# markdl/mtcp

Hardware: AMD Instinct MI355X
Metric: device-resident Gpkt/s + payload GB/s checksummed, 1/2/4/8 MI355X (higher is better)
Workload: dtype u8

## Files before the change

### mtcp_amd/csrc/rx_kernels.hpp

```cpp
#pragma once

#include <hip/hip_runtime.h>
#include <stdint.h>

#include <type_traits>

#include "../../include/mtcp_gpu.h"

namespace mg {

constexpr int kWave = 64;
constexpr int kBlock = 256;
constexpr int kWavesPerBlock = kBlock / kWave;
constexpr int kRssTableWords = 24 * 16;
constexpr int kSlotChunks = 8;
constexpr int kRow = 16;
constexpr int kUnroll = 6;

enum Mode : int { kRxChunk = 0, kRxPtrs = 1, kTxChunk = 2, kTxPtrs = 3 };
constexpr bool is_tx(int m) { return m == kTxChunk || m == kTxPtrs; }
enum Sched : int {
    kSchedRolled = 0,
    kSchedUnrolled = 3,
    kSchedSortedBase = 4,
    kSchedSortedEarly = 5,
    kSchedSorted = 6,
};

struct KParams {
    const uint8_t *buf;
    uint64_t buf_len;
    int64_t base_sub;
    const mtcp_gpu_desc *desc;
    const uint8_t *const *ptrs;
    const uint16_t *lens;
    uint32_t n;
    uint32_t off_shift;
    mtcp_gpu_result *out;
    const uint32_t *rss_tables;
    uint32_t rss_nq;
    uint32_t rss_endian;
    uint32_t *fill_count;
    uint32_t *bins;
    uint2 *tx_report;
    uint32_t *stamps;
    uint32_t rss_key[4];
    uint32_t compact;
};

typedef unsigned int v4u __attribute__((ext_vector_type(4)));

typedef __attribute__((address_space(1))) const v4u gv4u;
__device__ __forceinline__ v4u gload(uint64_t addr) { return *reinterpret_cast<gv4u *>(addr); }
__device__ __forceinline__ v4u gload_nt(uint64_t addr) {
    return __builtin_nontemporal_load(reinterpret_cast<gv4u *>(addr));
}
__device__ __forceinline__ uint4 gload4(uint64_t addr) {
    const v4u v = gload(addr);
    return make_uint4(v.x, v.y, v.z, v.w);
}

__device__ __forceinline__ uint32_t bswap16(uint32_t v) {
    return ((v & 0xFFu) << 8) | ((v >> 8) & 0xFFu);
}
__device__ __forceinline__ uint32_t bswap32(uint32_t v) { return __builtin_bswap32(v); }

__device__ __forceinline__ uint32_t halves(uint32_t d, uint32_t acc) {
    return __builtin_amdgcn_sad_u16(d, 0u, acc);
}
__device__ __forceinline__ uint32_t halves4(const v4u &v, uint32_t acc) {
    return halves(v.w, halves(v.z, halves(v.y, halves(v.x, acc))));
}

__device__ __forceinline__ uint32_t fold_csum(uint32_t s) {
    s = (s >> 16) + (s & 0xFFFFu);
    s += s >> 16;
    return (~s) & 0xFFFFu;
}

__device__ __forceinline__ uint32_t row_sum(uint32_t v) {
    v += (uint32_t)__builtin_amdgcn_update_dpp(0, (int)v, 0x111, 0xF, 0xF, true);
    v += (uint32_t)__builtin_amdgcn_update_dpp(0, (int)v, 0x112, 0xF, 0xF, true);
    v += (uint32_t)__builtin_amdgcn_update_dpp(0, (int)v, 0x114, 0xF, 0xF, true);
    v += (uint32_t)__builtin_amdgcn_update_dpp(0, (int)v, 0x118, 0xF, 0xF, true);
    return v;
}

__device__ __forceinline__ uint32_t shfl32(uint32_t v, int src) {
    return (uint32_t)__builtin_amdgcn_ds_bpermute(src << 2, (int)v);
}

__device__ __forceinline__ uint32_t row_bcast(uint32_t v, int i) {
#define MG_NB(n) case n: return (uint32_t)__builtin_amdgcn_update_dpp(0, (int)v, 0x150 + n, 0xF, 0xF, false)
    switch (i) {
        MG_NB(0); MG_NB(1); MG_NB(2); MG_NB(3); MG_NB(4); MG_NB(5); MG_NB(6); MG_NB(7);
        MG_NB(8); MG_NB(9); MG_NB(10); MG_NB(11); MG_NB(12); MG_NB(13); MG_NB(14);
        default: return (uint32_t)__builtin_amdgcn_update_dpp(0, (int)v, 0x15F, 0xF, 0xF, false);
    }
#undef MG_NB
}

__host__ __device__ __forceinline__ uint32_t hash_flow32(const uint32_t (&w)[3]) {
    uint32_t h = 0;
#pragma unroll
    for (int i = 0; i < 12; ++i) {
        h += (uint32_t)(int32_t)(int8_t)(uint8_t)(w[i >> 2] >> (8 * (i & 3)));
        h += h << 10;
        h ^= h >> 6;
    }
    h += h << 3;
    h ^= h >> 11;
    h += h << 15;
    return h;
}

__device__ __forceinline__ uint32_t hash_flow(const uint32_t (&w)[3]) {
    return hash_flow32(w) & (MTCP_GPU_NUM_BINS_FLOWS - 1);
}

__device__ __forceinline__ void flow_key(uint32_t saddr, uint32_t daddr, uint32_t ports, uint32_t (&w)[3]) {
    w[0] = daddr;
    w[1] = saddr;
    w[2] = (ports >> 16) | (ports << 16);
}

__device__ __forceinline__ uint32_t flow_bin(uint32_t saddr, uint32_t daddr, uint32_t ports,
                                             uint32_t verdict) {
    uint32_t w[3];
    flow_key(saddr, daddr, ports, w);
    return verdict == MTCP_GPU_V_TCP_OK ? hash_flow(w) : MTCP_GPU_FLOW_NONE;
}

template <int I0, int N, class F>
__device__ __forceinline__ void static_for(F &&f) {
    if constexpr (I0 < N) {
        f(std::integral_constant<int, I0>{});
        static_for<I0 + 1, N>(f);
    }
}

constexpr int kHdRows = 4 * kSlotChunks;
constexpr int kHdStride = kWave + 1;
struct WaveLds {
    uint32_t hd[kHdRows * kHdStride];
    uint32_t sum[kWave + 1];
    uint4 info[kWave];
};

struct Pkt {
    uint32_t verdict = MTCP_GPU_V_BAD_DESC;
    uint32_t eth_type = 0, ip_len = 0, ihl_doff = 0, ip_csum = 0, tcp_csum = 0;
    uint32_t saddr = 0, daddr = 0, ports = 0, seq = 0, ack = 0, window = 0, flags = 0;
    uint32_t payload_len = 0;
    uint32_t T = 0, s_ip = 0, ip_check = 0;
    uint32_t seg_len = 0;
    uint32_t tcheck = 0;
    bool tcp_entry = false;
    bool need_sum = false;
    bool icmp = false;
};

template <int MODE, class PD, class IPSUM, class SW, class SWB>
__device__ __forceinline__ Pkt parse_head(PD pd, IPSUM ipsum, SW sw, SWB swb, uint32_t L,
                                          bool desc_ok) {
    Pkt k;
    uint32_t h[7];
#pragma unroll
    for (int i = 3; i < 7; ++i) h[i] = pd(i);
    const uint32_t d0 = h[3];
    if (!desc_ok) return k;
    k.verdict = MTCP_GPU_V_TRUNCATED;
    if (L < 14) return k;
    k.eth_type = bswap16(d0 & 0xFFFFu);
    if (k.eth_type != 0x0800u) {
        k.verdict = k.eth_type == 0x0806u ? MTCP_GPU_V_ARP : MTCP_GPU_V_ETH_OTHER;
        return k;
    }
    if (L < 18) return k;
    k.ip_len = bswap16(h[4] & 0xFFFFu);
    const uint32_t ihl = (d0 >> 16) & 0xFu;
    k.ihl_doff = ihl;
    const uint32_t ver = (d0 >> 20) & 0xFu;
    if (!is_tx(MODE) && k.ip_len < 20) {
        k.verdict = MTCP_GPU_V_IP_SHORT;
        return k;
    }
    if (L < 14 + 4 * (ihl > 4 ? ihl : 1)) return k;
    if (ihl >= 5) k.s_ip = ipsum(ihl);
    k.ip_check = h[6] & 0xFFFFu;
    k.ip_csum = ihl <= 4 ? (d0 >> 16) : fold_csum(k.s_ip);
    const uint32_t proto = h[5] >> 24;
    k.T = 14 + 4 * ihl;
    bool tcp_entry = false;
    if (is_tx(MODE)) {
        tcp_entry = ver == 4 && ihl >= 5 && proto == 6 && L >= k.T + 20;
        k.verdict = MTCP_GPU_V_ETH_OTHER;
    } else if (k.ip_csum != 0) {
        k.verdict = MTCP_GPU_V_IP_CSUM_BAD;
    } else if (ver != 4) {
        k.verdict = MTCP_GPU_V_IP_VERSION;
    } else if (proto == 1) {
        k.verdict = MTCP_GPU_V_ICMP;
        if (14 + k.ip_len <= L) {
            if (k.ip_len >= 4 * ihl) {
                k.icmp = k.need_sum = true;
                k.seg_len = k.payload_len = k.ip_len - 4 * ihl;
            } else {
                k.tcp_csum = 0xFFFFu;
            }
        }
    } else if (proto != 6) {
        k.verdict = MTCP_GPU_V_IP_PROTO_OTHER;
    } else if (L >= k.T + 16) {
        tcp_entry = true;
    }
    if (tcp_entry) {
        const uint32_t tw = (k.T - 2) >> 2;
        const uint32_t e3 = pd(tw + 3), e4 = pd(tw + 4);
        const uint32_t doff = (e3 >> 20) & 0xFu;
        k.tcp_entry = true;
        k.saddr = sw(6);
        k.daddr = sw(7);
        k.ports = sw(tw);
        k.seq = swb(tw + 1);
        k.ack = swb(tw + 2);
        k.window = bswap16(e4 & 0xFFFFu);
        k.flags = e3 >> 24;
        k.tcheck = e4 >> 16;
        k.ihl_doff = ihl | (doff << 4);
        if (is_tx(MODE)) {
            if (doff >= 5 && k.ip_len >= 4 * (ihl + doff) && 14 + k.ip_len <= L) {
                k.need_sum = true;
                k.seg_len = k.ip_len - 4 * ihl;
            }
        } else if (k.ip_len < ((ihl + doff) << 2)) {
            k.verdict = MTCP_GPU_V_TCP_LEN_BAD;
        } else {
            k.payload_len = k.ip_len - ((ihl + doff) << 2);
            if (14 + k.ip_len <= L) {
                k.need_sum = true;
                k.seg_len = k.ip_len - 4 * ihl;
            }
        }
    }
    return k;
}

template <int MODE, class PD, class IPSUM, class SW, class SWB>
__device__ __forceinline__ bool parse_common(PD pd, IPSUM ipsum, SW sw, SWB swb, uint32_t L,
                                             bool desc_ok, Pkt &k) {
    if constexpr (is_tx(MODE)) {
        return false;
    } else {
        const uint32_t d0 = pd(3), h4 = pd(4), h5 = pd(5);
        const uint32_t ipl = bswap16(h4 & 0xFFFFu);
        if (!(desc_ok && L >= 50 && (d0 & 0xFFFFFFu) == 0x450008u && (h5 >> 24) == 6u && ipl >= 20u))
            return false;
        const uint32_t s_ip = ipsum(5u);
        if (fold_csum(s_ip) != 0) return false;
        const uint32_t e3 = pd(11), e4 = pd(12);
        const uint32_t doff = (e3 >> 20) & 0xFu, hlen = (5 + doff) << 2;
        const bool len_bad = ipl < hlen;
        k.verdict = len_bad ? MTCP_GPU_V_TCP_LEN_BAD : MTCP_GPU_V_TRUNCATED;
        k.eth_type = 0x0800u;
        k.ip_len = ipl;
        k.ihl_doff = 5u | (doff << 4);
        k.ip_csum = 0;
        k.s_ip = s_ip;
        k.ip_check = pd(6) & 0xFFFFu;
        k.T = 34;
        k.tcp_entry = true;
        k.saddr = sw(6);
        k.daddr = sw(7);
        k.ports = sw(8);
        k.seq = swb(9);
        k.ack = swb(10);
        k.window = bswap16(e4 & 0xFFFFu);
        k.flags = e3 >> 24;
        k.tcheck = e4 >> 16;
        k.payload_len = len_bad ? 0u : ipl - hlen;
        k.need_sum = !len_bad && 14 + ipl <= L;
        k.seg_len = k.need_sum ? ipl - 20 : 0u;
        k.icmp = false;
        k.tcp_csum = 0;
        return true;
    }
}

template <int MODE, class PD, class IPSUM, class SW, class SWB>
__device__ __forceinline__ Pkt parse_head_wave(PD pd, IPSUM ipsum, SW sw, SWB swb, uint32_t L,
                                               bool desc_ok) {
    Pkt k;
    if (parse_common<MODE>(pd, ipsum, sw, swb, L, desc_ok, k)) return k;
    return parse_head<MODE>(pd, ipsum, sw, swb, L, desc_ok);
}

template <int MODE, class PD, class IPSUM, class SW, class SWB>
__device__ __forceinline__ Pkt parse_head_sel(PD pd, IPSUM ipsum, SW sw, SWB swb, uint32_t L,
                                          bool desc_ok) {
    constexpr bool tx = is_tx(MODE);
    const uint32_t d0 = pd(3), h4 = pd(4), h5 = pd(5), h6 = pd(6);
    const uint32_t eth = bswap16(d0 & 0xFFFFu);
    const uint32_t ipl = bswap16(h4 & 0xFFFFu);
    const uint32_t ihl = (d0 >> 16) & 0xFu, ver = (d0 >> 20) & 0xFu;
    const uint32_t proto = h5 >> 24;
    const uint32_t T = 14 + 4 * ihl;
    const bool ok14 = desc_ok && L >= 14;
    const bool isip = ok14 && eth == 0x0800u;
    const bool ok18 = isip && L >= 18;
    const bool shrt = !tx && ipl < 20;
    const bool okhdr = ok18 && !shrt && L >= 14 + 4 * (ihl > 4 ? ihl : 1);
    const uint32_t s_ip = ipsum(ihl);
    const uint32_t ip_csum = ihl <= 4 ? (d0 >> 16) : fold_csum(s_ip);
    const bool ip_good = okhdr && ip_csum == 0 && ver == 4;
    const uint32_t tw = (T - 2) >> 2;
    const uint32_t e3 = pd(tw + 3), e4 = pd(tw + 4);
    const uint32_t doff = (e3 >> 20) & 0xFu;
    const bool tcp_entry = tx ? okhdr && ver == 4 && ihl >= 5 && proto == 6 && L >= T + 20
                              : ip_good && proto == 6 && L >= T + 16;
    const uint32_t hlen = (ihl + doff) << 2;
    const bool in_frame = 14 + ipl <= L;
    const bool len_bad = !tx && tcp_entry && ipl < hlen;
    const bool icmp_in = !tx && ip_good && proto == 1 && in_frame;
    const bool icmp = icmp_in && ipl >= 4 * ihl;
    const bool tcp_sum = tx ? tcp_entry && doff >= 5 && ipl >= hlen && in_frame
                            : tcp_entry && !len_bad && in_frame;

    uint32_t v = MTCP_GPU_V_TRUNCATED;
    if (!tx) {
        v = len_bad ? MTCP_GPU_V_TCP_LEN_BAD : v;
        v = ip_good && proto != 6 ? MTCP_GPU_V_IP_PROTO_OTHER : v;
        v = ip_good && proto == 1 ? MTCP_GPU_V_ICMP : v;
        v = okhdr && ip_csum == 0 && ver != 4 ? MTCP_GPU_V_IP_VERSION : v;
        v = okhdr && ip_csum != 0 ? MTCP_GPU_V_IP_CSUM_BAD : v;
        v = ok18 && shrt ? MTCP_GPU_V_IP_SHORT : v;
    } else {
        v = okhdr ? MTCP_GPU_V_ETH_OTHER : v;
    }
    v = ok14 && !isip ? (eth == 0x0806u ? MTCP_GPU_V_ARP : MTCP_GPU_V_ETH_OTHER) : v;
    v = desc_ok ? v : MTCP_GPU_V_BAD_DESC;

    Pkt k;
    k.verdict = v;
    k.eth_type = ok14 ? eth : 0u;
    k.ip_len = ok18 ? ipl : 0u;
    k.ihl_doff = ok18 ? ihl | (tcp_entry ? doff << 4 : 0u) : 0u;
    k.s_ip = okhdr && ihl >= 5 ? s_ip : 0u;
    k.ip_check = okhdr ? h6 & 0xFFFFu : 0u;
    k.ip_csum = okhdr ? ip_csum : 0u;
    k.T = okhdr ? T : 0u;
    k.tcp_entry = tcp_entry;
    k.saddr = tcp_entry ? sw(6) : 0u;
    k.daddr = tcp_entry ? sw(7) : 0u;
    k.ports = tcp_entry ? sw(tw) : 0u;
    k.seq = tcp_entry ? swb(tw + 1) : 0u;
    k.ack = tcp_entry ? swb(tw + 2) : 0u;
    k.window = tcp_entry ? bswap16(e4 & 0xFFFFu) : 0u;
    k.flags = tcp_entry ? e3 >> 24 : 0u;
    k.tcheck = tcp_entry ? e4 >> 16 : 0u;
    k.icmp = icmp;
    k.need_sum = tcp_sum || icmp;
    k.seg_len = k.need_sum ? ipl - 4 * ihl : 0u;
    k.payload_len = icmp ? ipl - 4 * ihl
                  : !tx && tcp_entry && !len_bad ? ipl - hlen : 0u;
    k.tcp_csum = icmp_in && !icmp ? 0xFFFFu : 0u;
    return k;
}

template <int MODE>
__device__ __forceinline__ void finish_seg(Pkt &k, uint32_t seg) {
    uint32_t s = seg;
    if (is_tx(MODE)) s -= k.tcheck;
    if (!k.icmp) {
        s += (k.saddr & 0xFFFFu) + (k.saddr >> 16);
        s += (k.daddr & 0xFFFFu) + (k.daddr >> 16);
        s += bswap16(k.seg_len);
        s += 0x0600u;
    }
    k.tcp_csum = fold_csum(s);
    if (!is_tx(MODE) && !k.icmp)
        k.verdict = k.tcp_csum ? MTCP_GPU_V_TCP_CSUM_BAD : MTCP_GPU_V_TCP_OK;
}

template <int MODE, int S, bool COMMON = false, bool ALIGNED = false>
__device__ __forceinline__ Pkt parse_finish(const uint32_t *raw, uint32_t sum, uint64_t p,
                                            uint32_t L, uint32_t nch, bool desc_ok) {
    const uint32_t sh = (uint32_t)(p & 15);
    const uint32_t a = sh >> 2, fb = 8 * (sh & 3);
    auto pd = [&](uint32_t i) -> uint32_t {
        if constexpr (ALIGNED) return raw[(a + i) * S];
        return __builtin_amdgcn_alignbit(raw[(a + i + 1) * S], raw[(a + i) * S], fb);
    };
    auto ipsum = [&](uint32_t ihl) -> uint32_t {
        uint32_t s_ip = pd(3) >> 16, lo_last = 0;
#pragma unroll
        for (int j = 1; j < 16; ++j) {
            const uint32_t w = pd(3 + j);
            s_ip = halves(j < (int)ihl ? w : 0u, s_ip);
            lo_last = j == (int)ihl ? w & 0xFFFFu : lo_last;
        }
        return s_ip + lo_last;
    };
    auto sw = [&](uint32_t i) -> uint32_t { return __builtin_amdgcn_alignbit(pd(i + 1), pd(i), 16); };
    auto swb = [&](uint32_t i) -> uint32_t { return bswap32(sw(i)); };
    Pkt k;
    if (!COMMON || !parse_common<MODE>(pd, ipsum, sw, swb, L, desc_ok, k))
        k = parse_head_sel<MODE>(pd, ipsum, sw, swb, L, desc_ok);
    if (k.need_sum) {
        uint32_t s_out = k.s_ip + (pd(3) & 0xFFFFu);
        s_out = halves(pd(2), halves(pd(1), halves(pd(0), s_out)));
#pragma unroll
        for (uint32_t i = 0; i < 3; ++i)
            if (i < a) s_out = halves(raw[i * S], s_out);
        if (!ALIGNED && (sh & 2)) s_out += raw[a * S] & 0xFFFFu;
        const uint64_t p16 = p & ~15ull;
        const uint64_t e_abs = p + 14 + k.ip_len;
        const uint64_t end = p16 + 16ull * nch;
        const uint32_t te = (uint32_t)(e_abs & 15);
        uint64_t cstart = e_abs & ~15ull;
        if (te) {
            uint4 w;
            if (cstart + 16 == end) {
                const uint32_t *t = raw + 4 * (kSlotChunks - 1) * S;
                w = make_uint4(t[0], t[S], t[2 * S], t[3 * S]);
            } else {
                w = gload4(cstart);
            }
            const uint32_t wv[4] = {w.x, w.y, w.z, w.w};
#pragma unroll
            for (int i = 0; i < 4; ++i) {
                const int drop = (int)te - 4 * i;
                const uint32_t m = drop <= 0 ? 0xFFFFFFFFu : drop >= 4 ? 0u : (0xFFFFFFFFu << (8 * drop));
                s_out = halves(wv[i] & m, s_out);
            }
            cstart += 16;
        }
        for (; cstart < end; cstart += 16) {
            const uint4 w = gload4(cstart);
            s_out = halves(w.w, halves(w.z, halves(w.y, halves(w.x, s_out))));
        }
        finish_seg<MODE>(k, sum - s_out);
    }
    return k;
}

__device__ __forceinline__ void pack_record(const Pkt &k, uint32_t rss_hash, uint32_t rss_queue,
                                            uint32_t (&r)[10]) {
    r[0] = k.saddr;
    r[1] = k.daddr;
    r[2] = k.ports;
    r[3] = k.seq;
    r[4] = k.ack;
    r[5] = k.window | (k.ip_len << 16);
    r[6] = k.ip_csum | (k.tcp_csum << 16);
    r[7] = rss_hash;
    r[8] = k.payload_len | (k.ihl_doff << 16) | (k.flags << 24);
    r[9] = k.verdict | (rss_queue << 8) | (k.eth_type << 16);
}

__device__ __forceinline__ void pack_compact(const Pkt &k, uint32_t rss_hash, uint32_t rss_queue,
                                             uint32_t (&r)[4]) {
    r[0] = rss_hash;
    r[1] = k.ip_csum | (k.tcp_csum << 16);
    r[2] = k.payload_len | (k.ip_len << 16);
    r[3] = k.ihl_doff | (k.flags << 8) | (k.verdict << 16) | (rss_queue << 24);
}

__device__ __forceinline__ void store_record(const KParams &kp, uint32_t rec, const Pkt &k,
                                             uint32_t rss_hash, uint32_t rss_queue) {
    if (kp.compact) {
        uint32_t c[4];
        pack_compact(k, rss_hash, rss_queue, c);
        reinterpret_cast<uint4 *>(kp.out)[rec] = make_uint4(c[0], c[1], c[2], c[3]);
    } else {
        uint32_t r[10];
        pack_record(k, rss_hash, rss_queue, r);
        uint2 *o = reinterpret_cast<uint2 *>(kp.out + rec);
#pragma unroll
        for (int i = 0; i < 5; ++i) o[i] = make_uint2(r[2 * i], r[2 * i + 1]);
    }
}

__device__ __forceinline__ uint32_t toeplitz_tables(const uint32_t *tab, uint32_t saddr,
                                                    uint32_t daddr, uint32_t ports) {
    uint32_t hh = 0;
#pragma unroll
    for (int b = 0; b < 4; ++b) {
        const uint32_t sb = (saddr >> (8 * b)) & 0xFFu;
        const uint32_t db = (daddr >> (8 * b)) & 0xFFu;
        const uint32_t pb = (ports >> (8 * b)) & 0xFFu;
        hh ^= tab[((2 * b) << 4) | (sb >> 4)] ^ tab[((2 * b + 1) << 4) | (sb & 15)];
        hh ^= tab[((8 + 2 * b) << 4) | (db >> 4)] ^ tab[((9 + 2 * b) << 4) | (db & 15)];
        hh ^= tab[((16 + 2 * b) << 4) | (pb >> 4)] ^ tab[((17 + 2 * b) << 4) | (pb & 15)];
    }
    return hh;
}

__device__ __forceinline__ uint32_t rss_core(uint32_t hh, uint32_t nq, uint32_t endian) {
    uint32_t m = hh & 0x7Fu;
    if (endian) m ^= 3u;
    return m % nq;
}

struct Frame {
    uint64_t p;
    uint32_t L;
    bool ok, live;
    uint64_t p16;
    uint32_t nch;
    uint32_t r_nch, r_lo, r_hi;
};

struct Trip {
    int i;
    uint32_t c0, nj;
    uint64_t base;
    uint32_t col;
    uint32_t skip = 0;
    uint32_t k = 0, ntrip = 0;
};

template <int MODE, bool RSS, int SCHED, bool LALIGN = false, int ABL = 0, int DEFER = 8, int B = 8,
          bool NT = true, int U = 6, bool REV = false, bool STAMP = false, int PRIO = 0,
          int WPB = kWavesPerBlock, int XSKIP = 0, bool CMP = false, int WPE = 2, bool COOP = true>
__global__ __launch_bounds__(kWave * WPB) __attribute__((amdgpu_waves_per_eu(WPE))) void rx_kernel(KParams kp) {
#ifndef MTCP_GPU_TESTING
    static_assert(ABL == 0 && !STAMP && XSKIP == 0,
                  "rx_kernel's ABL / STAMP / XSKIP variants need a -DMTCP_GPU_TESTING build (tools/)");
#endif
    uint64_t t_start = 0;
    if constexpr (STAMP) t_start = __builtin_amdgcn_s_memrealtime();
    if constexpr ((PRIO & 3) > 0) {
        if (blockIdx.x >= gridDim.x / 2) __builtin_amdgcn_s_setprio(PRIO & 3);
    }
    __shared__ uint32_t rss_lds[RSS ? kRssTableWords : 1];
    __shared__ WaveLds lds[WPB];
    if constexpr (RSS) {
        for (int i = threadIdx.x; i < kRssTableWords; i += kWave * WPB) rss_lds[i] = kp.rss_tables[i];
        __syncthreads();
    }

    const uint32_t lane = threadIdx.x & (kWave - 1);
    const uint32_t row = lane >> 4, rlane = lane & (kRow - 1);
    const uint32_t wib = threadIdx.x >> 6;
    const uint32_t wave = blockIdx.x * WPB + wib;
    const uint32_t nwaves = gridDim.x * WPB;
    WaveLds &wl = lds[wib];
    const uint32_t pass_pkts = nwaves * kWave;
    auto map = [&](uint32_t l) -> uint32_t {
        return B == kWave ? wave * kWave + l : (l / B) * (nwaves * B) + wave * B + (l % B);
    };
    const uint32_t lane_off = map(lane);
    bool xskip_wave = false;
    if constexpr (XSKIP != 0) {
        const uint32_t xcc = (uint32_t)__builtin_amdgcn_s_getreg((3 << 11) | 20) & 1u;
        xskip_wave = XSKIP > 0 ? xcc == 1u : xcc == 0u;
    }
    const uint64_t safe = (uint64_t)(uintptr_t)(MODE == kRxPtrs ? (const void *)kp.out
                                                               : (const void *)kp.buf);
    auto lane_pkt = [&](uint32_t g0, bool &live) -> uint32_t {
        live = g0 + lane_off < kp.n;
        return g0 + lane_off;
    };

    constexpr bool kCoop = B == 8 && MODE != kRxPtrs && SCHED == 3 && COOP;
    __shared__ uint64_t coop_a[kCoop ? 2 : 1][kCoop ? WPB * kWave : 1];
    uint32_t coop_buf = 0;

    const uint32_t cq = wib * kWave + lane, cj = cq / (8 * WPB), cidx = cq % (8 * WPB);
    const uint32_t coop_off = cj * (nwaves * 8) + blockIdx.x * (8 * WPB) + cidx;
    const uint32_t coop_slot = (cidx / 8) * kWave + cj * 8 + (cidx % 8);
    uint64_t raw_a = 0;
    uint32_t raw_b = 0;
    uint64_t cv_a = 0;
    auto fetch = [&](uint32_t g0) {
        if constexpr (kCoop) {
            const uint32_t kk = g0 + coop_off;
            if (kk < kp.n) cv_a = *reinterpret_cast<const uint64_t *>(kp.desc + kk);
            return;
        }
        bool live;
        const uint32_t k = lane_pkt(g0, live);
        if (live) {
            if constexpr (MODE == kRxPtrs) {
                raw_a = (uint64_t)(uintptr_t)kp.ptrs[k];
                raw_b = kp.lens[k];
            } else {
                raw_a = *reinterpret_cast<const uint64_t *>(kp.desc + k);
            }
        }
    };
    auto exchange = [&]() {
        if constexpr (kCoop) {
            coop_a[coop_buf][coop_slot] = cv_a;
            __syncthreads();
            raw_a = coop_a[coop_buf][wib * kWave + lane];
            coop_buf ^= 1u;
        }
    };
    auto decode = [&](uint32_t g0) -> Frame {
        Frame f;
        bool live;
        (void)lane_pkt(g0, live);
        f.live = live;
        if constexpr (XSKIP != 0) {
            if (xskip_wave && g0 + pass_pkts >= kp.n && lane >= (uint32_t)(kWave - (XSKIP > 0 ? XSKIP : -XSKIP)))
                f.live = false;
        }
        f.p = safe;
        f.L = 0;
        f.ok = false;
        if (f.live) {
            if constexpr (MODE == kRxPtrs) {
                f.L = raw_b;
                f.ok = raw_a != 0 && (raw_a & 1) == 0;
                if (f.ok) f.p = raw_a;
            } else {
                const uint32_t off = (uint32_t)raw_a;
                f.L = (uint32_t)(raw_a >> 32) & 0xFFFFu;
                const int64_t pos = (int64_t)((uint64_t)off << kp.off_shift) - kp.base_sub;
                f.ok = pos >= 0 && (pos & 1) == 0 && (uint64_t)pos + f.L <= kp.buf_len;
                if (f.ok) f.p = safe + (uint64_t)pos;
            }
        }
        f.p16 = f.p & ~15ull;
        f.nch = f.ok && f.L ? (uint32_t)((((f.p + f.L + 15) & ~15ull) - f.p16) >> 4) : 0u;
        const int src = 4 * (int)rlane + (int)row;
        f.r_nch = shfl32(f.nch, src);
        f.r_lo = shfl32((uint32_t)f.p16, src);
        f.r_hi = shfl32((uint32_t)(f.p16 >> 32), src);
        return f;
    };

    auto line_align = [&](Trip &t) {
        t.skip = 0;
        if constexpr (LALIGN) {
            if (t.nj > (uint32_t)(U * kRow)) {
                t.skip = (uint32_t)((t.base & 127) >> 4);
                t.base -= 16ull * t.skip;
                t.nj += t.skip;
            }
        }
    };
    auto enter_round = [&](const Frame &f, Trip &t, int ii) {
        t.i = ii;
        t.col = 4 * (uint32_t)ii + row;
        t.nj = row_bcast(f.r_nch, ii);
        t.base = ((uint64_t)row_bcast(f.r_hi, ii) << 32) | row_bcast(f.r_lo, ii);
        t.c0 = 0;
        line_align(t);
        if constexpr (REV) {
            t.k = 0;
            t.ntrip = (t.nj + U * kRow - 1) / (U * kRow);
            if ((row & 1) && t.ntrip > 1) t.c0 = (t.ntrip - 1) * (U * kRow);
        }
    };
    auto rev_step = [&](Trip &t) {
        ++t.k;
        t.c0 = t.k >= t.ntrip ? t.nj
               : (row & 1) ? (t.ntrip - 1 - t.k) * (U * kRow) : t.k * (U * kRow);
    };
    auto advance = [&](const Frame &f, Trip &t) -> bool {
        if (__ballot(t.c0 + U * kRow < t.nj)) {
            t.c0 += U * kRow;
            return true;
        }
        for (int ii = t.i + 1; ii < kWave / 4; ++ii) {
            enter_round(f, t, ii);
            if (__ballot(t.nj != 0)) return true;
        }
        t.nj = 0;
        return false;
    };
    auto first_trip = [&](const Frame &f, Trip &t) -> bool {
        enter_round(f, t, 0);
        return __ballot(t.nj != 0) || advance(f, t);
    };
    auto issue = [&](const Trip &t, v4u (&x)[U]) {
#pragma unroll
        for (int u = 0; u < U; ++u) {
            const uint32_t c = t.c0 + u * kRow + rlane;
            const uint32_t cc = c < t.nj ? c : (t.nj ? t.nj - 1 : 0u);
            x[u] = NT ? gload_nt(t.base + 16ull * cc) : gload(t.base + 16ull * cc);
        }
    };
    auto consume = [&](const Trip &t, const v4u (&x)[U], uint32_t &acc) {
        const uint32_t j = t.col;
        const uint32_t c_hd = rlane - t.skip;
        if (ABL < 2 && t.c0 == 0 && c_hd < kSlotChunks - 1) {
            uint32_t *d = wl.hd + 4 * c_hd * kHdStride + j;
            d[0] = x[0].x; d[kHdStride] = x[0].y;
            d[2 * kHdStride] = x[0].z; d[3 * kHdStride] = x[0].w;
        }
#pragma unroll
        for (int u = 0; u < U; ++u) {
            const uint32_t c = t.c0 + u * kRow + rlane;
            const uint32_t s = halves4(x[u], 0u);
            acc += (ABL >= 3 || c - t.skip < t.nj - t.skip) ? s : 0u;
            if (ABL < 2 && c == t.nj - 1) {
                uint32_t *d = wl.hd + 4 * (kSlotChunks - 1) * kHdStride + j;
                d[0] = x[u].x; d[kHdStride] = x[u].y;
                d[2 * kHdStride] = x[u].z; d[3 * kHdStride] = x[u].w;
            }
        }
    };

    constexpr uint32_t kSmallChunks = 4;
    constexpr uint32_t kQuads = kWave / 4;
    uint32_t pre_nL = 0, pre_nS = 0;
    auto prepare = [&](const Frame &fr, uint32_t &nL, uint32_t &nS) {
        const bool big = fr.nch > kSmallChunks, sml = fr.nch != 0 && !big;
        const uint64_t mb = __ballot(big), ms = __ballot(sml);
        nL = (uint32_t)__popcll(mb);
        nS = (uint32_t)__popcll(ms);
        const uint64_t below = (1ull << lane) - 1;
        const uint4 e = make_uint4((uint32_t)fr.p16, (uint32_t)(fr.p16 >> 32), fr.nch, lane);
        if (big) wl.info[__popcll(mb & below)] = e;
        if (sml) wl.info[kWave - 1 - __popcll(ms & below)] = e;
    };
    auto big_trip = [&](uint32_t nL, uint32_t ii, Trip &t) {
        const uint32_t r = 4 * ii + row;
        t.i = (int)ii;
        t.c0 = 0;
        t.skip = 0;
        t.nj = 0;
        t.base = safe;
        t.col = kWave;
        if (r < nL) {
            const uint4 e = wl.info[r];
            t.base = ((uint64_t)e.y << 32) | e.x;
            t.nj = e.z;
            t.col = e.w;
            line_align(t);
        }
    };
    auto small_trip = [&](uint32_t nS, uint32_t ii, Trip &t) {
        const uint32_t r = kQuads * ii + (lane >> 2);
        t.i = (int)ii;
        t.c0 = 0;
        t.skip = 0;
        t.nj = 0;
        t.base = safe;
        t.col = kWave;
        if (r < nS) {
            const uint4 e = wl.info[kWave - 1 - r];
            t.base = ((uint64_t)e.y << 32) | e.x;
            t.nj = e.z;
            t.col = e.w;
        }
    };
    auto small_load = [&](const Trip &t) -> v4u {
        const uint32_t q = lane & 3;
        const uint32_t cc = q < t.nj ? q : (t.nj ? t.nj - 1 : 0u);
        return NT && SCHED < 5 ? gload_nt(t.base + 16ull * cc) : gload(t.base + 16ull * cc);
    };
    auto small_finish = [&](const Trip &t, const v4u &v) {
        const uint32_t q = lane & 3;
        uint32_t s4 = q < t.nj ? halves4(v, 0u) : 0u;
        s4 += (uint32_t)__builtin_amdgcn_update_dpp(0, (int)s4, 0xB1, 0xF, 0xF, false);
        s4 += (uint32_t)__builtin_amdgcn_update_dpp(0, (int)s4, 0x4E, 0xF, 0xF, false);
        if (q == 0) wl.sum[t.col] = s4;
        if (q < t.nj) {
            uint32_t *d = wl.hd + 4 * q * kHdStride + t.col;
            d[0] = v.x; d[kHdStride] = v.y; d[2 * kHdStride] = v.z; d[3 * kHdStride] = v.w;
        }
        if (q + 1 == t.nj) {
            uint32_t *d = wl.hd + 4 * (kSlotChunks - 1) * kHdStride + t.col;
            d[0] = v.x; d[kHdStride] = v.y; d[2 * kHdStride] = v.z; d[3 * kHdStride] = v.w;
        }
    };

    constexpr int kDefer = MODE == kTxChunk ? 0 : DEFER;
    constexpr int RW = CMP ? 4 : 10, HW = CMP ? 5 : 10;
    uint32_t keep[kDefer > 0 ? kDefer : 1][HW];
    uint32_t held = 0;
    uint32_t last_g0 = 0;
    uint8_t *const out_b = reinterpret_cast<uint8_t *>(kp.out);
    auto flush = [&]() {
        if constexpr (kDefer > 0) {
            static_assert(B % 2 == 0, "16 B pieces need runs of an even number of records");
            constexpr uint32_t kRunDw = B * RW, kRunPieces = kRunDw / 4;
            uint32_t *stg = reinterpret_cast<uint32_t *>(&wl.hd[0]);
#pragma unroll
            for (int q = 0; q < kDefer; ++q) {
                if ((uint32_t)q < held) {
                    const uint32_t gq = last_g0 - (uint32_t)q * pass_pkts;
                    uint2 *st = reinterpret_cast<uint2 *>(stg) + lane * (RW / 2);
#pragma unroll
                    for (int i = 0; i < RW / 2; ++i) st[i] = make_uint2(keep[q][2 * i], keep[q][2 * i + 1]);
#pragma unroll
                    for (uint32_t pc = lane; pc < kWave * RW / 4; pc += kWave) {
                        const uint32_t run = pc / kRunPieces, w = pc % kRunPieces;
                        const uint32_t first = gq + map(run * B);
                        const uint32_t r0 = first + (4 * w) / RW, r1 = first + (4 * w + 2) / RW;
                        const uint4 v = *reinterpret_cast<const uint4 *>(stg + run * kRunDw + 4 * w);
                        uint8_t *dst = out_b + (uint64_t)first * (4 * RW) + 16 * w;
                        if (r1 < kp.n) {
                            *reinterpret_cast<uint4 *>(dst) = v;
                        } else if (r0 < kp.n) {
                            *reinterpret_cast<uint2 *>(dst) = make_uint2(v.x, v.y);
                        }
                    }
                    if (kp.bins) {
                        bool live;
                        const uint32_t rec = lane_pkt(gq, live);
                        if (live)
                            kp.bins[rec] = CMP ? keep[q][HW - 1]
                                               : flow_bin(keep[q][0], keep[q][1], keep[q][2], keep[q][9] & 0xFFu);
                    }
                }
            }
            held = 0;
        }
    };

    auto push = [&](const uint32_t (&r)[HW], uint32_t g0) {
        if constexpr (kDefer > 0) {
            if (held == (uint32_t)kDefer) flush();
#pragma unroll
            for (int q = kDefer - 1; q > 0; --q)
#pragma unroll
                for (int i = 0; i < HW; ++i) keep[q][i] = keep[q - 1][i];
#pragma unroll
            for (int i = 0; i < HW; ++i) keep[0][i] = r[i];
            last_g0 = g0;
            ++held;
        }
    };

    constexpr int kTxDefer = MODE == kTxChunk && DEFER > 0 ? DEFER : 0;
    uint32_t tkeep[kTxDefer > 0 ? kTxDefer : 1][4];
    uint32_t tx_held = 0;
    auto tx_write = [&](const uint32_t (&w)[4]) {
        if (w[3]) {
            uint16_t *q16 = reinterpret_cast<uint16_t *>(((uint64_t)w[1] << 32) | w[0]);
            q16[12] = (uint16_t)w[2];
            q16[(w[3] + 16) >> 1] = (uint16_t)(w[2] >> 16);
        }
    };
    auto tx_flush = [&]() {
        if constexpr (kTxDefer > 0) {
#pragma unroll
            for (int q = 0; q < kTxDefer; ++q)
                if ((uint32_t)q < tx_held) tx_write(tkeep[q]);
            tx_held = 0;
        }
    };
    auto tx_push = [&](const uint32_t (&w)[4]) {
        if constexpr (kTxDefer > 0) {
            if (tx_held == (uint32_t)kTxDefer) tx_flush();
#pragma unroll
            for (int q = kTxDefer - 1; q > 0; --q)
#pragma unroll
                for (int i = 0; i < 4; ++i) tkeep[q][i] = tkeep[q - 1][i];
#pragma unroll
            for (int i = 0; i < 4; ++i) tkeep[0][i] = w[i];
            ++tx_held;
        }
    };

    fetch(0);
    exchange();
    v4u X[U], Y[U];
    Trip pre;
    bool have_pre = false;
    Trip sa, sb;
    v4u va, vb;
    bool have_pre_small = false;
    for (uint32_t g0 = 0; g0 < kp.n; g0 += pass_pkts) {
        if constexpr ((PRIO & 4) != 0) {
            if (g0 == 4 * pass_pkts) __builtin_amdgcn_s_setprio(0);
        }
        const Frame f = decode(g0);
        if (!__ballot(f.live)) break;
        fetch(g0 + pass_pkts);
        const uint32_t k = g0 + lane_off;
        const bool live = f.live, desc_ok = f.ok;
        const uint64_t p = f.p;
        const uint32_t L = f.L, nch = f.nch;
        const bool has_next = g0 + pass_pkts < kp.n;

        if constexpr (SCHED >= 4) {
            uint32_t nL, nS;
            if (!have_pre) prepare(f, nL, nS);
            else nL = pre_nL, nS = pre_nS;
            const uint32_t RL = (nL + 3) / 4, RS = (nS + kQuads - 1) / kQuads;
            uint32_t acc = 0;
            auto finish_big = [&](Trip &t, const v4u (&cb)[U]) {
                consume(t, cb, acc);
                while (__ballot(t.c0 + U * kRow < t.nj)) {
                    t.c0 += U * kRow;
                    v4u Z[U];
                    issue(t, Z);
                    consume(t, Z, acc);
                }
                acc = row_sum(acc);
                if (rlane == kRow - 1) wl.sum[t.col] = acc;
                acc = 0;
            };
            if constexpr (SCHED >= 5) {
                if (have_pre_small) {
                } else if (RL > 0 && !have_pre) {
                    Trip t0;
                    big_trip(nL, 0, t0);
                    issue(t0, X);
                    pre = t0;
                    have_pre = true;
                }
                if (!have_pre_small) {
                    small_trip(nS, 0, sa);
                    small_trip(nS, 1, sb);
                    va = small_load(sa);
                    vb = small_load(sb);
                }
                have_pre_small = false;
            }
            if (RL > 0) {
                Trip cur, nxt;
                if (have_pre) {
                    cur = pre;
                } else {
                    big_trip(nL, 0, cur);
                    issue(cur, X);
                }
                for (uint32_t i = 0; i < RL; i += 2) {
                    if (i + 1 < RL) {
                        big_trip(nL, i + 1, nxt);
                        issue(nxt, Y);
                    }
                    finish_big(cur, X);
                    if (i + 1 >= RL) break;
                    if (i + 2 < RL) {
                        big_trip(nL, i + 2, cur);
                        issue(cur, X);
                    }
                    finish_big(nxt, Y);
                }
            }
            have_pre = false;
            uint32_t s0 = 0;
            if constexpr (SCHED >= 5) {
                if (RS > 0) {
                    small_finish(sa, va);
                    small_finish(sb, vb);
                }
                s0 = 2;
            }
            for (uint32_t i = s0; i < RS; i += 2) {
                Trip a, b;
                small_trip(nS, i, a);
                small_trip(nS, i + 1, b);
                const v4u va = small_load(a), vb = small_load(b);
                small_finish(a, va);
                small_finish(b, vb);
            }
            if (has_next) {
                exchange();
                const Frame fn = decode(g0 + pass_pkts);
                prepare(fn, pre_nL, pre_nS);
                if constexpr (SCHED == 6) {
                    small_trip(pre_nS, 0, sa);
                    small_trip(pre_nS, 1, sb);
                    va = small_load(sa);
                    vb = small_load(sb);
                    have_pre_small = true;
                }
                if (pre_nL) {
                    big_trip(pre_nL, 0, pre);
                    issue(pre, X);
                    have_pre = true;
                }
            }
        } else if constexpr (SCHED == 3) {
            uint32_t acc = 0;
            static_for<0, kWave / 4>([&](auto I) {
                constexpr int i = decltype(I)::value;
                Trip t;
                enter_round(f, t, i);
                if (i > 0 || !have_pre) issue(t, X);
                consume(t, X, acc);
                if constexpr (REV) {
                    while (__ballot(t.k + 1 < t.ntrip)) {
                        rev_step(t);
                        issue(t, X);
                        consume(t, X, acc);
                    }
                } else {
                    while (__ballot(t.c0 + U * kRow < t.nj)) {
                        t.c0 += U * kRow;
                        issue(t, X);
                        consume(t, X, acc);
                    }
                }
                acc = row_sum(acc);
                if (rlane == kRow - 1) wl.sum[4 * i + (int)row] = acc;
                acc = 0;
            });
            have_pre = false;
            if (has_next) {
                exchange();
                const Frame fn = decode(g0 + pass_pkts);
                Trip n;
                enter_round(fn, n, 0);
                issue(n, X);
                have_pre = true;
            }
        } else {
            Trip cur;
            bool have;
            if (have_pre) {
                cur = pre;
                have = true;
            } else {
                have = first_trip(f, cur);
                issue(cur, X);
            }
            have_pre = false;
            uint32_t acc = 0;
            while (have) {
                Trip n = cur;
                const bool more = advance(f, n);
                consume(cur, X, acc);
                if (!more || n.i != cur.i) {
                    acc = row_sum(acc);
                    if (rlane == kRow - 1) wl.sum[4 * cur.i + (int)row] = acc;
                    acc = 0;
                }
                if (!more) break;
                issue(n, X);
                cur = n;
            }
            if (has_next) {
                Trip n;
                exchange();
                const Frame fn = decode(g0 + pass_pkts);
                if (__ballot(fn.live) && first_trip(fn, n)) {
                    issue(n, X);
                    pre = n;
                    have_pre = true;
                }
            }
        }

        if constexpr (ABL >= 1) {
            if constexpr (kDefer > 0) {
                uint32_t r[HW] = {};
                r[0] = wl.sum[lane];
                push(r, g0);
            } else if (live && wl.sum[lane] == 0x12345678u) {
                kp.out[k].saddr = wl.sum[lane];
            }
            continue;
        }
        const Pkt pk = parse_finish<MODE, kHdStride>(wl.hd + lane, wl.sum[lane], p, L, nch, desc_ok);
        uint32_t rss_hash = 0, rss_queue = 0;
        if constexpr (RSS) {
            if (pk.tcp_entry) {
                rss_hash = toeplitz_tables(rss_lds, pk.saddr, pk.daddr, pk.ports);
                rss_queue = rss_core(rss_hash, kp.rss_nq, kp.rss_endian);
            }
        }

        if constexpr (MODE == kTxChunk) {
            uint32_t fill[4] = {0, 0, 0, 0};
            if (live && pk.need_sum) {
                const uint32_t ipc = fold_csum(pk.s_ip - pk.ip_check);
                fill[0] = (uint32_t)p;
                fill[1] = (uint32_t)(p >> 32);
                fill[2] = ipc | (pk.tcp_csum << 16);
                fill[3] = pk.T;
                if (kp.fill_count) atomicAdd(kp.fill_count, 1u);
            }
            if constexpr (kTxDefer > 0) {
                tx_push(fill);
            } else {
                tx_write(fill);
            }
        } else {
            uint32_t r[HW];
            if constexpr (CMP) {
                uint32_t c[4];
                pack_compact(pk, rss_hash, rss_queue, c);
#pragma unroll
                for (int i = 0; i < 4; ++i) r[i] = c[i];
                r[4] = kp.bins ? flow_bin(pk.saddr, pk.daddr, pk.ports, pk.verdict) : 0u;
            } else {
                pack_record(pk, rss_hash, rss_queue, r);
            }
            if constexpr (kDefer > 0) {
                push(r, g0);
            } else {
                uint2 *st = reinterpret_cast<uint2 *>(wl.hd) + lane * (RW / 2);
#pragma unroll
                for (int i = 0; i < RW / 2; ++i) st[i] = make_uint2(r[2 * i], r[2 * i + 1]);
                const uint2 *src = reinterpret_cast<const uint2 *>(wl.hd);
#pragma unroll
                for (uint32_t i = 0; i < RW / 2; ++i) {
                    const uint32_t q = i * kWave + lane;
                    const uint32_t rec = g0 + map(q / (RW / 2));
                    if (rec < kp.n)
                        reinterpret_cast<uint2 *>(out_b + (uint64_t)rec * (4 * RW))[q % (RW / 2)] = src[q];
                }
                if (kp.bins && live)
                    kp.bins[k] = CMP ? r[HW - 1] : flow_bin(r[0], r[1], r[2], r[9] & 0xFFu);
            }
        }
    }
    flush();
    tx_flush();
    if constexpr (STAMP) {
        __builtin_amdgcn_s_waitcnt(0);
        const uint64_t t_end = __builtin_amdgcn_s_memrealtime();
        if (lane == 0) {
            uint32_t *st = kp.stamps + 4 * wave;
            st[0] = (uint32_t)t_start;
            st[1] = (uint32_t)t_end;
            st[2] = (uint32_t)__builtin_amdgcn_s_getreg((3 << 11) | 20);
            st[3] = (uint32_t)__builtin_amdgcn_s_getreg((31 << 11) | 4);
        }
    }
}

}
```

Measured before the change: 6579.

## Add quota-based last-pass dealing and trim empty rounds in unrolled schedule

Adds a DEAL template option that redistributes the final pass's packets across blocks by a per-XCD quota table, changing the pass iteration to a PassId abstraction and making held-record flushes aware of dealt passes. Separately, the unrolled SCHED==3 path now counts how many 4-packet rounds actually contain frames and runs a rolled loop over only those rounds, skipping empty trailing rounds. It also recomputes lane and coop indices from threadIdx with asm barriers and pins rss_nq to a scalar register. DEAL is off by default and testing-only, but the round-trimming path is active and adds a dynamic loop in place of the fully unrolled sequence, which may cost register or scheduling quality.

Measured after the change: 6569. About the same (-0.2%).

```diff
diff --git a/mtcp_amd/csrc/rx_kernels.hpp b/mtcp_amd/csrc/rx_kernels.hpp
--- a/mtcp_amd/csrc/rx_kernels.hpp
+++ b/mtcp_amd/csrc/rx_kernels.hpp
@@ -46,6 +46,7 @@
     uint32_t *stamps;
     uint32_t rss_key[4];
     uint32_t compact;
+    uint8_t quota[8];
 };
 
 typedef unsigned int v4u __attribute__((ext_vector_type(4)));
@@ -520,13 +521,19 @@
     uint32_t k = 0, ntrip = 0;
 };
 
+struct PassId {
+    uint32_t g, nj;
+};
+constexpr uint32_t kWholePass = ~0u;
+
 template <int MODE, bool RSS, int SCHED, bool LALIGN = false, int ABL = 0, int DEFER = 8, int B = 8,
           bool NT = true, int U = 6, bool REV = false, bool STAMP = false, int PRIO = 0,
-          int WPB = kWavesPerBlock, int XSKIP = 0, bool CMP = false, int WPE = 2, bool COOP = true>
+          int WPB = kWavesPerBlock, int XSKIP = 0, bool CMP = false, int WPE = 2, bool COOP = true,
+          bool DEAL = false>
 __global__ __launch_bounds__(kWave * WPB) __attribute__((amdgpu_waves_per_eu(WPE))) void rx_kernel(KParams kp) {
 #ifndef MTCP_GPU_TESTING
-    static_assert(ABL == 0 && !STAMP && XSKIP == 0,
-                  "rx_kernel's ABL / STAMP / XSKIP variants need a -DMTCP_GPU_TESTING build (tools/)");
+    static_assert(ABL == 0 && !STAMP && XSKIP == 0 && !DEAL,
+                  "rx_kernel's ABL / STAMP / XSKIP / DEAL variants need a -DMTCP_GPU_TESTING build (tools/)");
 #endif
     uint64_t t_start = 0;
     if constexpr (STAMP) t_start = __builtin_amdgcn_s_memrealtime();
@@ -550,7 +557,54 @@
     auto map = [&](uint32_t l) -> uint32_t {
         return B == kWave ? wave * kWave + l : (l / B) * (nwaves * B) + wave * B + (l % B);
     };
-    const uint32_t lane_off = map(lane);
+    static_assert(!DEAL || (MODE == kRxChunk && SCHED == 3 && !LALIGN && B == 8 && WPB == 4 && COOP &&
+                            DEFER > 0 && XSKIP == 0),
+                  "DEAL is for the unrolled chunk schedule with runs of 8 and held records");
+    bool deal_on = false;
+    uint32_t deal_g = 0, deal_q = 0, g_last = 0;
+    if constexpr (DEAL) {
+        uint32_t sum = 0, before = 0;
+        bool even = true;
+#pragma unroll
+        for (uint32_t m = 0; m < 8; ++m) {
+            sum += kp.quota[m];
+            before += m < (blockIdx.x & 7u) ? kp.quota[m] : 0u;
+            deal_q = m == (blockIdx.x & 7u) ? kp.quota[m] : deal_q;
+            even = even && kp.quota[m] == 8;
+        }
+        deal_on = !even && sum == 64 && gridDim.x % 8 == 0 && kp.n != 0 && kp.n % pass_pkts == 0;
+        if (deal_on) {
+            g_last = kp.n - pass_pkts;
+            deal_g = g_last + 32 * (64 * (blockIdx.x >> 3) + before);
+        }
+    }
+    auto dealt = [&](const PassId &c) -> bool {
+        if constexpr (DEAL) return c.nj != kWholePass;
+        return false;
+    };
+    auto first_pass = [&]() -> PassId {
+        if constexpr (DEAL) {
+            if (deal_on && g_last == 0) return PassId{deal_g, deal_q < 8 ? deal_q : 8u};
+        }
+        return PassId{0, kWholePass};
+    };
+    auto next_pass = [&](const PassId &c, PassId &n) -> bool {
+        if constexpr (DEAL) {
+            if (deal_on) {
+                if (dealt(c)) {
+                    const bool mini = c.g == deal_g && deal_q > 8;
+                    n = PassId{deal_g + 256, mini ? deal_q - 8 : 0u};
+                    return mini;
+                }
+                if (c.g + pass_pkts >= g_last) {
+                    n = PassId{deal_g, deal_q < 8 ? deal_q : 8u};
+                    return deal_q != 0;
+                }
+            }
+        }
+        n = PassId{c.g + pass_pkts, kWholePass};
+        return n.g < kp.n;
+    };
     bool xskip_wave = false;
     if constexpr (XSKIP != 0) {
         const uint32_t xcc = (uint32_t)__builtin_amdgcn_s_getreg((3 << 11) | 20) & 1u;
@@ -558,29 +612,50 @@
     }
     const uint64_t safe = (uint64_t)(uintptr_t)(MODE == kRxPtrs ? (const void *)kp.out
                                                                : (const void *)kp.buf);
-    auto lane_pkt = [&](uint32_t g0, bool &live) -> uint32_t {
-        live = g0 + lane_off < kp.n;
-        return g0 + lane_off;
+    auto pkt_of = [&](const PassId &c, bool &live, uint32_t ln, uint32_t wb) -> uint32_t {
+        if (dealt(c)) {
+            live = (ln >> 3) < c.nj;
+            return c.g + 32 * (ln >> 3) + 8 * wb + (ln & 7u);
+        }
+        const uint32_t wv = blockIdx.x * WPB + wb;
+        const uint32_t k = c.g + (B == kWave ? wv * kWave + ln : (ln / B) * (nwaves * B) + wv * B + (ln % B));
+        live = k < kp.n;
+        return k;
+    };
+    auto lane_pkt = [&](const PassId &c, bool &live) -> uint32_t {
+        uint32_t t = threadIdx.x;
+        asm volatile("" : "+v"(t));
+        return pkt_of(c, live, t & (kWave - 1), t >> 6);
     };
 
     constexpr bool kCoop = B == 8 && MODE != kRxPtrs && SCHED == 3 && COOP;
     __shared__ uint64_t coop_a[kCoop ? 2 : 1][kCoop ? WPB * kWave : 1];
     uint32_t coop_buf = 0;
 
-    const uint32_t cq = wib * kWave + lane, cj = cq / (8 * WPB), cidx = cq % (8 * WPB);
-    const uint32_t coop_off = cj * (nwaves * 8) + blockIdx.x * (8 * WPB) + cidx;
-    const uint32_t coop_slot = (cidx / 8) * kWave + cj * 8 + (cidx % 8);
+    auto coop_entry = [&](uint32_t &cj, uint32_t &cidx) -> uint32_t {
+        uint32_t cq = threadIdx.x;
+        asm volatile("" : "+v"(cq));
+        cj = cq / (8 * WPB);
+        cidx = cq % (8 * WPB);
+        return cq;
+    };
     uint64_t raw_a = 0;
     uint32_t raw_b = 0;
     uint64_t cv_a = 0;
-    auto fetch = [&](uint32_t g0) {
+    auto fetch = [&](const PassId &c) {
         if constexpr (kCoop) {
-            const uint32_t kk = g0 + coop_off;
+            uint32_t cj, cidx;
+            coop_entry(cj, cidx);
+            if (dealt(c)) {
+                if (cj < c.nj) cv_a = *reinterpret_cast<const uint64_t *>(kp.desc + c.g + 32 * cj + cidx);
+                return;
+            }
+            const uint32_t kk = c.g + cj * (nwaves * 8) + blockIdx.x * (8 * WPB) + cidx;
             if (kk < kp.n) cv_a = *reinterpret_cast<const uint64_t *>(kp.desc + kk);
             return;
         }
         bool live;
-        const uint32_t k = lane_pkt(g0, live);
+        const uint32_t k = lane_pkt(c, live);
         if (live) {
             if constexpr (MODE == kRxPtrs) {
                 raw_a = (uint64_t)(uintptr_t)kp.ptrs[k];
@@ -592,19 +667,21 @@
     };
     auto exchange = [&]() {
         if constexpr (kCoop) {
-            coop_a[coop_buf][coop_slot] = cv_a;
+            uint32_t cj, cidx;
+            const uint32_t cq = coop_entry(cj, cidx);
+            coop_a[coop_buf][(cidx / 8) * kWave + cj * 8 + (cidx % 8)] = cv_a;
             __syncthreads();
-            raw_a = coop_a[coop_buf][wib * kWave + lane];
+            raw_a = coop_a[coop_buf][cq];
             coop_buf ^= 1u;
         }
     };
-    auto decode = [&](uint32_t g0) -> Frame {
+    auto decode = [&](const PassId &c) -> Frame {
         Frame f;
         bool live;
-        (void)lane_pkt(g0, live);
+        (void)lane_pkt(c, live);
         f.live = live;
         if constexpr (XSKIP != 0) {
-            if (xskip_wave && g0 + pass_pkts >= kp.n && lane >= (uint32_t)(kWave - (XSKIP > 0 ? XSKIP : -XSKIP)))
+            if (xskip_wave && c.g + pass_pkts >= kp.n && lane >= (uint32_t)(kWave - (XSKIP > 0 ? XSKIP : -XSKIP)))
                 f.live = false;
         }
         f.p = safe;
@@ -775,35 +852,50 @@
     uint32_t keep[kDefer > 0 ? kDefer : 1][HW];
     uint32_t held = 0;
     uint32_t last_g0 = 0;
+    uint32_t held_deal = 0;
+    auto held_pass = [&](int q) -> PassId {
+        if constexpr (DEAL) {
+            const PassId main{deal_g, deal_q < 8 ? deal_q : 8u}, mini{deal_g + 256, deal_q - 8};
+            if (q == 0 && held_deal == 1) return main;
+            if (q == 0 && held_deal >= 2) return mini;
+            if (q == 1 && held_deal == 3) return main;
+            const uint32_t nd = held_deal == 3 ? 2u : held_deal ? 1u : 0u;
+            return PassId{last_g0 - ((uint32_t)q - nd) * pass_pkts, kWholePass};
+        }
+        return PassId{last_g0 - (uint32_t)q * pass_pkts, kWholePass};
+    };
     uint8_t *const out_b = reinterpret_cast<uint8_t *>(kp.out);
     auto flush = [&]() {
         if constexpr (kDefer > 0) {
             static_assert(B % 2 == 0, "16 B pieces need runs of an even number of records");
             constexpr uint32_t kRunDw = B * RW, kRunPieces = kRunDw / 4;
             uint32_t *stg = reinterpret_cast<uint32_t *>(&wl.hd[0]);
+            uint32_t ft = threadIdx.x;
+            asm volatile("" : "+v"(ft));
+            const uint32_t fl = ft & (kWave - 1), fw = ft >> 6;
 #pragma unroll
             for (int q = 0; q < kDefer; ++q) {
                 if ((uint32_t)q < held) {
-                    const uint32_t gq = last_g0 - (uint32_t)q * pass_pkts;
-                    uint2 *st = reinterpret_cast<uint2 *>(stg) + lane * (RW / 2);
+                    const PassId cq = held_pass(q);
+                    uint2 *st = reinterpret_cast<uint2 *>(stg) + fl * (RW / 2);
 #pragma unroll
                     for (int i = 0; i < RW / 2; ++i) st[i] = make_uint2(keep[q][2 * i], keep[q][2 * i + 1]);
 #pragma unroll
-                    for (uint32_t pc = lane; pc < kWave * RW / 4; pc += kWave) {
+                    for (uint32_t pc = fl; pc < kWave * RW / 4; pc += kWave) {
                         const uint32_t run = pc / kRunPieces, w = pc % kRunPieces;
-                        const uint32_t first = gq + map(run * B);
+                        const uint32_t first = dealt(cq) ? cq.g + 32 * run + 8 * fw : cq.g + map(run * B);
                         const uint32_t r0 = first + (4 * w) / RW, r1 = first + (4 * w + 2) / RW;
                         const uint4 v = *reinterpret_cast<const uint4 *>(stg + run * kRunDw + 4 * w);
                         uint8_t *dst = out_b + (uint64_t)first * (4 * RW) + 16 * w;
-                        if (r1 < kp.n) {
+                        if (dealt(cq) ? run < cq.nj : r1 < kp.n) {
                             *reinterpret_cast<uint4 *>(dst) = v;
-                        } else if (r0 < kp.n) {
+                        } else if (!dealt(cq) && r0 < kp.n) {
                             *reinterpret_cast<uint2 *>(dst) = make_uint2(v.x, v.y);
                         }
                     }
                     if (kp.bins) {
                         bool live;
-                        const uint32_t rec = lane_pkt(gq, live);
+                        const uint32_t rec = pkt_of(cq, live, fl, fw);
                         if (live)
                             kp.bins[rec] = CMP ? keep[q][HW - 1]
                                                : flow_bin(keep[q][0], keep[q][1], keep[q][2], keep[q][9] & 0xFFu);
@@ -811,10 +903,11 @@
                 }
             }
             held = 0;
-        }
-    };
-
-    auto push = [&](const uint32_t (&r)[HW], uint32_t g0) {
+            held_deal = 0;
+        }
+    };
+
+    auto push = [&](const uint32_t (&r)[HW], const PassId &c) {
         if constexpr (kDefer > 0) {
             if (held == (uint32_t)kDefer) flush();
 #pragma unroll
@@ -823,7 +916,8 @@
                 for (int i = 0; i < HW; ++i) keep[q][i] = keep[q - 1][i];
 #pragma unroll
             for (int i = 0; i < HW; ++i) keep[0][i] = r[i];
-            last_g0 = g0;
+            if (dealt(c)) held_deal = c.g != deal_g ? (held_deal == 1 ? 3u : 2u) : 1u;
+            else last_g0 = c.g;
             ++held;
         }
     };
@@ -859,7 +953,8 @@
         }
     };
 
-    fetch(0);
+    PassId cur = first_pass();
+    fetch(cur);
     exchange();
     v4u X[U], Y[U];
     Trip pre;
@@ -867,18 +962,22 @@
     Trip sa, sb;
     v4u va, vb;
     bool have_pre_small = false;
-    for (uint32_t g0 = 0; g0 < kp.n; g0 += pass_pkts) {
+    PassId nxt{0, kWholePass};
+    bool has_next = false;
+    for (bool more = kp.n != 0; more; cur = nxt, more = has_next) {
         if constexpr ((PRIO & 4) != 0) {
-            if (g0 == 4 * pass_pkts) __builtin_amdgcn_s_setprio(0);
-        }
-        const Frame f = decode(g0);
+            if ((dealt(cur) ? g_last : cur.g) == 4 * pass_pkts) __builtin_amdgcn_s_setprio(0);
+        }
+        const Frame f = decode(cur);
         if (!__ballot(f.live)) break;
-        fetch(g0 + pass_pkts);
-        const uint32_t k = g0 + lane_off;
-        const bool live = f.live, desc_ok = f.ok;
+        has_next = next_pass(cur, nxt);
+        fetch(nxt);
+        bool live;
+        const uint32_t k = lane_pkt(cur, live);
+        live = f.live;
+        const bool desc_ok = f.ok;
         const uint64_t p = f.p;
         const uint32_t L = f.L, nch = f.nch;
-        const bool has_next = g0 + pass_pkts < kp.n;
 
         if constexpr (SCHED >= 4) {
             uint32_t nL, nS;
@@ -956,7 +1055,7 @@
             }
             if (has_next) {
                 exchange();
-                const Frame fn = decode(g0 + pass_pkts);
+                const Frame fn = decode(nxt);
                 prepare(fn, pre_nL, pre_nS);
                 if constexpr (SCHED == 6) {
                     small_trip(pre_nS, 0, sa);
@@ -972,34 +1071,59 @@
                 }
             }
         } else if constexpr (SCHED == 3) {
+            const uint64_t with_frame = __ballot(f.nch != 0);
+            const int rounds = with_frame ? (63 - __clzll(with_frame)) / 4 + 1 : 0;
             uint32_t acc = 0;
-            static_for<0, kWave / 4>([&](auto I) {
-                constexpr int i = decltype(I)::value;
-                Trip t;
-                enter_round(f, t, i);
-                if (i > 0 || !have_pre) issue(t, X);
-                consume(t, X, acc);
-                if constexpr (REV) {
-                    while (__ballot(t.k + 1 < t.ntrip)) {
-                        rev_step(t);
-                        issue(t, X);
-                        consume(t, X, acc);
-                    }
-                } else {
+            if (!REV && rounds < kWave / 4) {
+                for (int ii = 0; ii < (rounds ? rounds : 1); ++ii) {
+                    Trip t;
+                    t.i = ii;
+                    t.col = 4 * (uint32_t)ii + row;
+                    t.nj = shfl32(f.nch, (int)t.col);
+                    t.base = ((uint64_t)shfl32((uint32_t)(f.p16 >> 32), (int)t.col) << 32) |
+                             shfl32((uint32_t)f.p16, (int)t.col);
+                    t.c0 = 0;
+                    line_align(t);
+                    if (ii > 0 || !have_pre) issue(t, X);
+                    consume(t, X, acc);
                     while (__ballot(t.c0 + U * kRow < t.nj)) {
                         t.c0 += U * kRow;
                         issue(t, X);
                         consume(t, X, acc);
                     }
-                }
-                acc = row_sum(acc);
-                if (rlane == kRow - 1) wl.sum[4 * i + (int)row] = acc;
-                acc = 0;
-            });
+                    acc = row_sum(acc);
+                    if (rlane == kRow - 1) wl.sum[t.col] = acc;
+                    acc = 0;
+                }
+            } else {
+                static_for<0, kWave / 4>([&](auto I) {
+                    constexpr int i = decltype(I)::value;
+                    Trip t;
+                    enter_round(f, t, i);
+                    if (i > 0 || !have_pre) issue(t, X);
+                    consume(t, X, acc);
+                    if constexpr (REV) {
+                        while (__ballot(t.k + 1 < t.ntrip)) {
+                            rev_step(t);
+                            issue(t, X);
+                            consume(t, X, acc);
+                        }
+                    } else {
+                        while (__ballot(t.c0 + U * kRow < t.nj)) {
+                            t.c0 += U * kRow;
+                            issue(t, X);
+                            consume(t, X, acc);
+                        }
+                    }
+                    acc = row_sum(acc);
+                    if (rlane == kRow - 1) wl.sum[4 * i + (int)row] = acc;
+                    acc = 0;
+                });
+            }
             have_pre = false;
             if (has_next) {
                 exchange();
-                const Frame fn = decode(g0 + pass_pkts);
+                const Frame fn = decode(nxt);
                 Trip n;
                 enter_round(fn, n, 0);
                 issue(n, X);
@@ -1033,7 +1157,7 @@
             if (has_next) {
                 Trip n;
                 exchange();
-                const Frame fn = decode(g0 + pass_pkts);
+                const Frame fn = decode(nxt);
                 if (__ballot(fn.live) && first_trip(fn, n)) {
                     issue(n, X);
                     pre = n;
@@ -1046,7 +1170,7 @@
             if constexpr (kDefer > 0) {
                 uint32_t r[HW] = {};
                 r[0] = wl.sum[lane];
-                push(r, g0);
+                push(r, cur);
             } else if (live && wl.sum[lane] == 0x12345678u) {
                 kp.out[k].saddr = wl.sum[lane];
             }
@@ -1057,7 +1181,9 @@
         if constexpr (RSS) {
             if (pk.tcp_entry) {
                 rss_hash = toeplitz_tables(rss_lds, pk.saddr, pk.daddr, pk.ports);
-                rss_queue = rss_core(rss_hash, kp.rss_nq, kp.rss_endian);
+                uint32_t nq = kp.rss_nq;
+                if constexpr (SCHED == 3) asm volatile("" : "+s"(nq));
+                rss_queue = rss_core(rss_hash, nq, kp.rss_endian);
             }
         }
 
@@ -1088,7 +1214,7 @@
                 pack_record(pk, rss_hash, rss_queue, r);
             }
             if constexpr (kDefer > 0) {
-                push(r, g0);
+                push(r, cur);
             } else {
                 uint2 *st = reinterpret_cast<uint2 *>(wl.hd) + lane * (RW / 2);
 #pragma unroll
@@ -1097,7 +1223,7 @@
 #pragma unroll
                 for (uint32_t i = 0; i < RW / 2; ++i) {
                     const uint32_t q = i * kWave + lane;
-                    const uint32_t rec = g0 + map(q / (RW / 2));
+                    const uint32_t rec = cur.g + map(q / (RW / 2));
                     if (rec < kp.n)
                         reinterpret_cast<uint2 *>(out_b + (uint64_t)rec * (4 * RW))[q % (RW / 2)] = src[q];
                 }
```
